# can-lehmann/exprgrad

Hardware: AMD Instinct MI355X
Metric: GFLOP/s matmul 4096^3 f32 (1 GPU) (higher is better)
Workload: dtype f32

## Files before the change

exprgrad_amd/csrc/kernels/gemm_split_bf16.hip:

```cpp
#include <algorithm>
#include <cfloat>

#include "gemm_fused.hpp"
#include "../eg_internal.hpp"
#include "../switches.hpp"

namespace {

typedef __bf16 bf16x8 __attribute__((ext_vector_type(8)));
typedef float f32x4 __attribute__((ext_vector_type(4)));


struct SplitOperand {
  const float* src;
  long ld;
  long R;
  int kc;
  __bf16* dst;
};

__device__ __forceinline__ void unit_coords(const SplitOperand& o, long K, long u, long& r, long& chunk) {
  const long cpr = K / 8, t = u >> 6;
  const int l = (int)(u & 63);
  if (o.kc) {
    const long per = cpr / 4;
    r = (t / per) * 16 + (l >> 2);
    chunk = (t % per) * 4 + (l & 3);
  } else {
    const long per = cpr / 2;
    r = (t / per) * 32 + (l >> 1);
    chunk = (t % per) * 2 + (l & 1);
  }
}

__device__ __forceinline__ void load_unit(const SplitOperand& o, long r, long chunk, float (&x)[8]) {
  if (o.kc) {
    const f32x4* p = reinterpret_cast<const f32x4*>(o.src + r * o.ld + chunk * 8);
    const f32x4 v0 = __builtin_nontemporal_load(p), v1 = __builtin_nontemporal_load(p + 1);
#pragma unroll
    for (int j = 0; j < 4; ++j) {
      x[j] = v0[j];
      x[4 + j] = v1[j];
    }
  } else {
    const float* p = o.src + chunk * 8 * o.ld + r;
#pragma unroll
    for (int j = 0; j < 8; ++j) x[j] = __builtin_nontemporal_load(p + j * o.ld);
  }
}

__device__ __forceinline__ void split_unit(const SplitOperand& o, long K, long r, long chunk, const float (&x)[8], bool& bad) {
  bf16x8 h0, h1, h2;
#pragma unroll
  for (int j = 0; j < 8; ++j) {
    const float v = x[j];
    const __bf16 b0 = (__bf16)v;
    const float r1 = v - (float)b0;
    const __bf16 b1 = (__bf16)r1;
    const float f1 = (float)b1;
    const float r2 = r1 - f1;
    const __bf16 b2 = (__bf16)r2;
    const float f2 = (float)b2;
    bad |= !(r2 == f2);
    bad |= v != 0.f && __builtin_fabsf(v) < FLT_MIN;
    bad |= (f1 != 0.f && __builtin_fabsf(f1) < FLT_MIN) || (f2 != 0.f && __builtin_fabsf(f2) < FLT_MIN);
    h0[j] = b0;
    h1[j] = b1;
    h2[j] = b2;
  }
  const long plane = o.R * K;
  bf16x8* d = reinterpret_cast<bf16x8*>(o.dst + ((chunk >> 1) * o.R + r) * 16 + (chunk & 1) * 8);
  const long ps = plane / 8;
  d[0] = h0;
  d[ps] = h1;
  d[2 * ps] = h2;
}

constexpr int SPLIT_NT = 256;
constexpr int SPLIT_U = 2;

__global__ __launch_bounds__(SPLIT_NT) void split_planes_kernel(SplitOperand a, SplitOperand b, long K, long units_a, long units,
                                                              unsigned* flag, unsigned epoch) {
  constexpr long STEP = (long)SPLIT_NT * SPLIT_U;
  const long per = ((units + gridDim.x - 1) / gridDim.x + STEP - 1) / STEP * STEP;
  const long lo = (long)blockIdx.x * per, hi = lo + per < units ? lo + per : units;
  bool bad = false;
  for (long base = lo; base < hi; base += STEP) {
    float x[SPLIT_U][8];
    long r[SPLIT_U], c[SPLIT_U];
#pragma unroll
    for (int i = 0; i < SPLIT_U; ++i) {
      const long u = base + i * SPLIT_NT + threadIdx.x;
      if (u >= hi) continue;
      const bool in_a = u < units_a;
      unit_coords(in_a ? a : b, K, in_a ? u : u - units_a, r[i], c[i]);
      load_unit(in_a ? a : b, r[i], c[i], x[i]);
    }
#pragma unroll
    for (int i = 0; i < SPLIT_U; ++i) {
      const long u = base + i * SPLIT_NT + threadIdx.x;
      if (u >= hi) continue;
      split_unit(u < units_a ? a : b, K, r[i], c[i], x[i], bad);
    }
  }
  if (__builtin_expect(bad, 0)) *(volatile unsigned*)flag = epoch;
}


constexpr int BM = 256, BN = 256, WM = 128, WN = 64, NT = 512;
constexpr int STAGES = 3;
constexpr int PLANE_BYTES = BM * 16 * 2;
constexpr int STAGE_BYTES = 6 * PLANE_BYTES;
constexpr int LOADS = STAGE_BYTES / (NT * 16);

struct SplitGemmArgs {
  const __bf16* pa;
  const __bf16* pb;
  float* C;
  const float* bias;
  long M, N, K, ldc;
  int tiles_m, tiles_n;
  int accumulate;
  int skew;
  const unsigned* flag;
  unsigned epoch;
};

__device__ __forceinline__ int xcd_remap(int bid, int nwg) {
  constexpr int NXCD = 8;
  const int q = nwg / NXCD, r = nwg % NXCD;
  const int xcd = bid % NXCD, local = bid / NXCD;
  return (xcd < r ? xcd * (q + 1) : r * (q + 1) + (xcd - r) * q) + local;
}
__device__ __forceinline__ void tile_origin(int wgid, int tiles_m, int tiles_n, long& m_blk, long& n_blk) {
  constexpr int GROUP = 8;
  const int per_group = GROUP * tiles_n;
  const int first_m = (wgid / per_group) * GROUP;
  const int gsize = min(tiles_m - first_m, GROUP);
  const int in_group = wgid % per_group;
  m_blk = (long)(first_m + in_group % gsize) * BM;
  n_blk = (long)(in_group / gsize) * BN;
}

__device__ __forceinline__ const void* uniform_ptr(const void* p) {
  const unsigned long v = reinterpret_cast<unsigned long>(p);
  const unsigned lo = __builtin_amdgcn_readfirstlane((unsigned)v), hi = __builtin_amdgcn_readfirstlane((unsigned)(v >> 32));
  return reinterpret_cast<const void*>(((unsigned long)hi << 32) | lo);
}

constexpr int ROLE_LOAD_OWN = 1, ROLE_LOAD_PARTNER = 2, ROLE_READ_TOP = 4, ROLE_READ_AHEAD = 8;
constexpr int PARTNER = 4;

#ifdef EG_SPLIT_GEMM_STAMPS
constexpr int STAMP_BLOCKS = 1024;
__device__ unsigned long long g_split_stamps[STAMP_BLOCKS][8][4];
#define EG_STAMP(t)                                                                  \
  do {                                                                               \
    __builtin_amdgcn_sched_barrier(0);                                               \
    asm volatile("s_memtime %0\n\ts_waitcnt lgkmcnt(0)" : "=s"(t)::"memory"); \
    __builtin_amdgcn_sched_barrier(0);                                               \
  } while (0)
#else
#define EG_STAMP(t) \
  do {              \
  } while (0)
#endif

__global__ __launch_bounds__(NT) void split_gemm_kernel(SplitGemmArgs a) {
  if (*(volatile const unsigned*)a.flag == a.epoch) return;
  __shared__ __attribute__((aligned(16))) unsigned char lds[STAGES * STAGE_BYTES];

  const int tid = threadIdx.x, lane = tid & 63, wave = __builtin_amdgcn_readfirstlane(tid >> 6);
  const int wr = wave >> 2, wc = wave & 3;
  long m_blk, n_blk;
  tile_origin(xcd_remap(blockIdx.x, gridDim.x), a.tiles_m, a.tiles_n, m_blk, n_blk);

  const __amdgpu_buffer_rsrc_t ra = __builtin_amdgcn_make_buffer_rsrc(
      const_cast<void*>(uniform_ptr(a.pa + m_blk * 16)), (short)0, -1, 0x00020000);
  const __amdgpu_buffer_rsrc_t rb = __builtin_amdgcn_make_buffer_rsrc(
      const_cast<void*>(uniform_ptr(a.pb + n_blk * 16)), (short)0, -1, 0x00020000);
  const unsigned a_plane = (unsigned)(a.M * a.K * 2), b_plane = (unsigned)(a.N * a.K * 2);
  const unsigned a_ktile = (unsigned)(a.M * 32), b_ktile = (unsigned)(a.N * 32);
  const unsigned voff = (unsigned)lane * 16;

  auto pieces = [&](int kt, int s, int w) {
    unsigned char* st = lds + s * STAGE_BYTES + w * 1024;
    const unsigned at = (unsigned)kt * a_ktile + (unsigned)w * 1024, bt = (unsigned)kt * b_ktile + (unsigned)w * 1024;
#pragma unroll
    for (int i = 0; i < LOADS; ++i) {
      __attribute__((address_space(3))) void* dst = (__attribute__((address_space(3))) void*)(st + i * PLANE_BYTES);
      if (i < 3)
        __builtin_amdgcn_raw_ptr_buffer_load_lds(ra, dst, 16, voff, (unsigned)i * a_plane + at, 0, 0);
      else
        __builtin_amdgcn_raw_ptr_buffer_load_lds(rb, dst, 16, voff, (unsigned)(i - 3) * b_plane + bt, 0, 0);
    }
  };
  auto issue = [&](int kt, int s, int r) {
    if (r & ROLE_LOAD_OWN) pieces(kt, s, wave);
    if (r & ROLE_LOAD_PARTNER) pieces(kt, s, wave ^ PARTNER);
  };

  f32x4 acc[8][4];
#pragma unroll
  for (int i = 0; i < 8; ++i)
#pragma unroll
    for (int j = 0; j < 4; ++j)
#pragma unroll
      for (int r = 0; r < 4; ++r) acc[i][j][r] = 0.f;

  const int sel = lane >> 5;
  const int a_row = (wr * WM + (lane & 15)) * 32 + ((lane >> 4) & 1) * 16;
  const int b_row = 3 * PLANE_BYTES + (wc * WN + (lane & 15)) * 32 + ((lane >> 4) & 1) * 16;
  const int a01_off = a_row + sel * PLANE_BYTES, a02_off = a_row + 2 * sel * PLANE_BYTES;
  const int b21_off = b_row + (2 - sel) * PLANE_BYTES, b10_off = b_row + (1 - sel) * PLANE_BYTES, b00_off = b_row;

  bf16x8 fb21[4], fb10[4], fb00[4], fa01, fa02;
  auto read_head = [&](const unsigned char* st) {
#pragma unroll
    for (int j = 0; j < 4; ++j) {
      fb21[j] = *reinterpret_cast<const bf16x8*>(st + b21_off + j * 512);
      fb10[j] = *reinterpret_cast<const bf16x8*>(st + b10_off + j * 512);
      fb00[j] = *reinterpret_cast<const bf16x8*>(st + b00_off + j * 512);
    }
    fa01 = *reinterpret_cast<const bf16x8*>(st + a01_off);
    fa02 = *reinterpret_cast<const bf16x8*>(st + a02_off);
  };
#pragma unroll
  for (int j = 0; j < 4; ++j) fb21[j] = fb10[j] = fb00[j] = bf16x8{};
  fa01 = fa02 = bf16x8{};

  const int skew = a.skew;
  const int role = !skew ? ROLE_LOAD_OWN | ROLE_READ_TOP
                         : (wave & PARTNER) ? ROLE_LOAD_OWN | ROLE_LOAD_PARTNER | ROLE_READ_TOP : ROLE_READ_AHEAD;
  const int KT = (int)(a.K / 16);
  issue(0, 0, role);
  if (KT > 1) issue(1, 1, role);
  if (skew) {
    if (KT > 1) asm volatile("s_waitcnt vmcnt(12)" ::: "memory");
    else asm volatile("s_waitcnt vmcnt(0)" ::: "memory");
    __builtin_amdgcn_s_barrier();
    asm volatile("" ::: "memory");
    if (role & ROLE_READ_AHEAD) read_head(lds);
  }
#ifdef EG_SPLIT_GEMM_STAMPS
  unsigned long long t0 = 0, t1 = 0, t2 = 0, front = 0, body = 0, back = 0;
#endif
  int s = 0;
  for (int kt = 0; kt < KT; ++kt) {
    if (!skew && kt + 1 < KT) asm volatile("s_waitcnt vmcnt(6)" ::: "memory");
    else asm volatile("s_waitcnt vmcnt(0)" ::: "memory");
    __builtin_amdgcn_s_barrier();
    asm volatile("" ::: "memory");
#ifdef EG_SPLIT_GEMM_STAMPS
    EG_STAMP(t0);
    if (kt) back += t0 - t2;
#endif
    int r = role;
    asm volatile("" : "+s"(r));
    if (kt + 2 < KT) issue(kt + 2, s == 0 ? 2 : s - 1, r);
    const unsigned char* st = lds + s * STAGE_BYTES;
    if (r & ROLE_READ_TOP) read_head(st);
    EG_STAMP(t1);
    bf16x8 c01 = fa01, c02 = fa02;
#pragma unroll
    for (int i = 0; i < 8; ++i) {
      bf16x8 n01 = c01, n02 = c02;
      __builtin_amdgcn_sched_barrier(0);
      if (i + 1 < 8) {
        n01 = *reinterpret_cast<const bf16x8*>(st + a01_off + (i + 1) * 512);
        n02 = *reinterpret_cast<const bf16x8*>(st + a02_off + (i + 1) * 512);
      }
      __builtin_amdgcn_sched_barrier(0);
#pragma unroll
      for (int j = 0; j < 4; ++j) acc[i][j] = __builtin_amdgcn_mfma_f32_16x16x32_bf16(c01, fb21[j], acc[i][j], 0, 0, 0);
#pragma unroll
      for (int j = 0; j < 4; ++j) acc[i][j] = __builtin_amdgcn_mfma_f32_16x16x32_bf16(c01, fb10[j], acc[i][j], 0, 0, 0);
#pragma unroll
      for (int j = 0; j < 4; ++j) acc[i][j] = __builtin_amdgcn_mfma_f32_16x16x32_bf16(c02, fb00[j], acc[i][j], 0, 0, 0);
      c01 = n01;
      c02 = n02;
    }
    EG_STAMP(t2);
#ifdef EG_SPLIT_GEMM_STAMPS
    front += t1 - t0;
    body += t2 - t1;
#endif
    s = s == STAGES - 1 ? 0 : s + 1;
    if ((r & ROLE_READ_AHEAD) && kt + 1 < KT) read_head(lds + s * STAGE_BYTES);
  }
#ifdef EG_SPLIT_GEMM_STAMPS
  if (lane == 0 && blockIdx.x < STAMP_BLOCKS) {
    unsigned long long* o = g_split_stamps[blockIdx.x][wave];
    o[0] = front;
    o[1] = body;
    o[2] = back;
    o[3] = (unsigned long long)KT;
  }
#endif

  __syncthreads();
  float* park = reinterpret_cast<float*>(lds) + wave * 64 * WN;
  const int prow = lane >> 4, pc4 = (lane & 15) * 4;
  const long col = n_blk + wc * WN + pc4;
  f32x4 b4 = {0.f, 0.f, 0.f, 0.f};
  if (a.bias) b4 = *reinterpret_cast<const f32x4*>(a.bias + col);
#pragma unroll
  for (int h = 0; h < 2; ++h) {
#pragma unroll
    for (int i = 0; i < 4; ++i)
#pragma unroll
      for (int j = 0; j < 4; ++j)
#pragma unroll
        for (int r = 0; r < 4; ++r) park[(i * 16 + 4 * prow + r) * WN + j * 16 + (lane & 15)] = acc[4 * h + i][j][r];
    asm volatile("s_waitcnt lgkmcnt(0)" ::: "memory");
#pragma unroll
    for (int q = 0; q < 16; ++q) {
      const int row = 4 * q + prow;
      f32x4 v = *reinterpret_cast<const f32x4*>(park + row * WN + pc4);
      f32x4* c = reinterpret_cast<f32x4*>(a.C + (m_blk + wr * WM + h * 64 + row) * a.ldc + col);
      if (a.accumulate) v = *c + v;
      if (a.bias) v = v + b4;
      *c = v;
    }
    asm volatile("s_waitcnt lgkmcnt(0)" ::: "memory");
  }
}

inline bool aligned16(const void* p) { return (reinterpret_cast<uintptr_t>(p) & 15) == 0; }

constexpr size_t kPlaneCap = 1ull << 30;

}

namespace eg {
namespace gemm {

int sgemm_split(eg_ctx* ctx, int trans_a, int trans_b, long M, long N, long K, const float* A, long lda, const float* B, long ldb,
                float* C, long ldc, int accumulate, const float* bias) {
  if (!ctx || !A || !B || !C || M <= 0 || N <= 0 || K <= 0) return EG_ERR_UNSUPPORTED;
  if (lda < (trans_a ? M : K) || ldb < (trans_b ? K : N) || ldc < N) return EG_ERR_UNSUPPORTED;
  if (eg::sw::on("EG_NO_SPLIT_GEMM")) return EG_ERR_UNSUPPORTED;
  if (M % BM != 0 || N % BN != 0 || K % 32 != 0 || K < 2048) return EG_ERR_UNSUPPORTED;
  if ((M / BM) * (N / BN) < ctx->compute_units) return EG_ERR_UNSUPPORTED;
  const size_t plane_bytes = 6 * (size_t)(M + N) * (size_t)K;
  if (plane_bytes > kPlaneCap || 6 * (size_t)std::max(M, N) * (size_t)K >= (1ull << 31)) return EG_ERR_UNSUPPORTED;
  if (!aligned16(A) || !aligned16(B) || (!trans_a && lda % 4 != 0) || (trans_b && ldb % 4 != 0)) return EG_ERR_UNSUPPORTED;
  if (!aligned16(C) || ldc % 4 != 0 || (bias && !aligned16(bias))) return EG_ERR_UNSUPPORTED;
  if (!exact_single_launch(ctx, trans_a, trans_b, M, N, K, A, lda, B, ldb, C, ldc, bias)) return EG_ERR_UNSUPPORTED;

  int rc = eg::set_device(ctx);
  if (rc) return rc;
  if (!ctx->split_flag) {
    EG_HIP_CHECK(hipMalloc((void**)&ctx->split_flag, sizeof(unsigned)));
    EG_HIP_CHECK(hipMemset(ctx->split_flag, 0, sizeof(unsigned)));
  }
  rc = eg::ensure_workspace(ctx, plane_bytes);
  if (rc) return rc;
  if (++ctx->split_epoch == 0) ctx->split_epoch = 1;
  const unsigned epoch = ctx->split_epoch;

  __bf16* pa = static_cast<__bf16*>(ctx->workspace);
  __bf16* pb = pa + 3 * (size_t)M * K;
  const SplitOperand oa = {A, lda, M, trans_a ? 0 : 1, pa};
  const SplitOperand ob = {B, ldb, N, trans_b ? 1 : 0, pb};
  const long units_a = M * K / 8, units = (M + N) * K / 8;
  long blocks = (units + SPLIT_NT * SPLIT_U - 1) / (SPLIT_NT * SPLIT_U);
  if (blocks > 8L * ctx->compute_units) blocks = 8L * ctx->compute_units;
  hipLaunchKernelGGL(split_planes_kernel, dim3((unsigned)blocks), dim3(SPLIT_NT), 0, ctx->stream, oa, ob, K, units_a, units,
                     ctx->split_flag, epoch);
  EG_HIP_CHECK(hipGetLastError());

  SplitGemmArgs g = {};
  g.pa = pa;
  g.pb = pb;
  g.C = C;
  g.bias = bias;
  g.M = M;
  g.N = N;
  g.K = K;
  g.ldc = ldc;
  g.tiles_m = (int)(M / BM);
  g.tiles_n = (int)(N / BN);
  g.accumulate = accumulate;
  g.skew = eg::sw::present("EG_GEMM_NO_SKEW") ? 0 : 1;
  g.flag = ctx->split_flag;
  g.epoch = epoch;
  hipLaunchKernelGGL(split_gemm_kernel, dim3((unsigned)(g.tiles_m * g.tiles_n)), dim3(NT), 0, ctx->stream, g);
  EG_HIP_CHECK(hipGetLastError());

  return sgemm_exact(ctx, trans_a, trans_b, M, N, K, A, lda, B, ldb, C, ldc, accumulate, bias, ctx->split_flag, epoch);
}

}
}

#ifdef EG_SPLIT_GEMM_STAMPS
extern "C" int eg_debug_split_stamps(unsigned long long* dst, size_t count) {
  if (count > sizeof(g_split_stamps) / sizeof(unsigned long long)) return EG_ERR_UNSUPPORTED;
  EG_HIP_CHECK(hipDeviceSynchronize());
  EG_HIP_CHECK(hipMemcpyFromSymbol(dst, HIP_SYMBOL(g_split_stamps), count * sizeof(unsigned long long)));
  return 0;
}
#endif
```

Measured before the change: 255,000.

## Interleave A and B split work per block and vectorize bf16 splitting

Rewrites the split pass so each block gets a balanced, interleaved share of A and B work items instead of a contiguous unit range. Hot loads and conversions become cheaper: unit coordinates use 32-bit division, bf16 conversions run two lanes at a time, and the subnormal checks use the hardware class instruction. The aim is to balance memory traffic between the two operands (which have different access patterns) and trim ALU work in a bandwidth-bound preprocessing kernel. It also adds optional timestamp instrumentation behind a compile flag, plus shape checks that reject shapes the partition cannot handle.

```diff
diff --git a/exprgrad_amd/csrc/kernels/gemm_split_bf16.hip b/exprgrad_amd/csrc/kernels/gemm_split_bf16.hip
--- a/exprgrad_amd/csrc/kernels/gemm_split_bf16.hip
+++ b/exprgrad_amd/csrc/kernels/gemm_split_bf16.hip
@@ -2,6 +2,7 @@
 #include <cfloat>
 
 #include "gemm_fused.hpp"
+#include "split_partition.hpp"
 #include "../eg_internal.hpp"
 #include "../switches.hpp"
 
@@ -19,20 +20,6 @@
   __bf16* dst;
 };
 
-__device__ __forceinline__ void unit_coords(const SplitOperand& o, long K, long u, long& r, long& chunk) {
-  const long cpr = K / 8, t = u >> 6;
-  const int l = (int)(u & 63);
-  if (o.kc) {
-    const long per = cpr / 4;
-    r = (t / per) * 16 + (l >> 2);
-    chunk = (t % per) * 4 + (l & 3);
-  } else {
-    const long per = cpr / 2;
-    r = (t / per) * 32 + (l >> 1);
-    chunk = (t % per) * 2 + (l & 1);
-  }
-}
-
 __device__ __forceinline__ void load_unit(const SplitOperand& o, long r, long chunk, float (&x)[8]) {
   if (o.kc) {
     const f32x4* p = reinterpret_cast<const f32x4*>(o.src + r * o.ld + chunk * 8);
@@ -49,24 +36,31 @@
   }
 }
 
+typedef __bf16 bf16x2 __attribute__((ext_vector_type(2)));
+typedef float f32x2 __attribute__((ext_vector_type(2)));
+constexpr unsigned kSubnormal = (1u << 4) | (1u << 7);
+
 __device__ __forceinline__ void split_unit(const SplitOperand& o, long K, long r, long chunk, const float (&x)[8], bool& bad) {
   bf16x8 h0, h1, h2;
 #pragma unroll
-  for (int j = 0; j < 8; ++j) {
-    const float v = x[j];
-    const __bf16 b0 = (__bf16)v;
-    const float r1 = v - (float)b0;
-    const __bf16 b1 = (__bf16)r1;
-    const float f1 = (float)b1;
-    const float r2 = r1 - f1;
-    const __bf16 b2 = (__bf16)r2;
-    const float f2 = (float)b2;
-    bad |= !(r2 == f2);
-    bad |= v != 0.f && __builtin_fabsf(v) < FLT_MIN;
-    bad |= (f1 != 0.f && __builtin_fabsf(f1) < FLT_MIN) || (f2 != 0.f && __builtin_fabsf(f2) < FLT_MIN);
-    h0[j] = b0;
-    h1[j] = b1;
-    h2[j] = b2;
+  for (int j = 0; j < 8; j += 2) {
+    const f32x2 v = {x[j], x[j + 1]};
+    const bf16x2 b0 = __builtin_convertvector(v, bf16x2);
+    const f32x2 r1 = v - __builtin_convertvector(b0, f32x2);
+    const bf16x2 b1 = __builtin_convertvector(r1, bf16x2);
+    const f32x2 f1 = __builtin_convertvector(b1, f32x2);
+    const f32x2 r2 = r1 - f1;
+    const bf16x2 b2 = __builtin_convertvector(r2, bf16x2);
+    const f32x2 f2 = __builtin_convertvector(b2, f32x2);
+#pragma unroll
+    for (int e = 0; e < 2; ++e) {
+      bad |= !(r2[e] == f2[e]);
+      bad |= __builtin_amdgcn_classf(v[e], kSubnormal);
+      bad |= __builtin_amdgcn_classf(f1[e], kSubnormal) || __builtin_amdgcn_classf(f2[e], kSubnormal);
+      h0[j + e] = b0[e];
+      h1[j + e] = b1[e];
+      h2[j + e] = b2[e];
+    }
   }
   const long plane = o.R * K;
   bf16x8* d = reinterpret_cast<bf16x8*>(o.dst + ((chunk >> 1) * o.R + r) * 16 + (chunk & 1) * 8);
@@ -76,34 +70,54 @@
   d[2 * ps] = h2;
 }
 
-constexpr int SPLIT_NT = 256;
+constexpr int SPLIT_NT = eg::gemm::kSplitItemUnits;
 constexpr int SPLIT_U = 2;
 
-__global__ __launch_bounds__(SPLIT_NT) void split_planes_kernel(SplitOperand a, SplitOperand b, long K, long units_a, long units,
+#ifdef EG_SPLIT_PASS_STAMPS
+constexpr int PASS_STAMP_BLOCKS = 4096;
+__device__ unsigned long long g_pass_stamps[PASS_STAMP_BLOCKS][2];
+#endif
+
+__global__ __launch_bounds__(SPLIT_NT) void split_planes_kernel(SplitOperand a, SplitOperand b, long K, eg::gemm::SplitShares shares,
                                                               unsigned* flag, unsigned epoch) {
-  constexpr long STEP = (long)SPLIT_NT * SPLIT_U;
-  const long per = ((units + gridDim.x - 1) / gridDim.x + STEP - 1) / STEP * STEP;
-  const long lo = (long)blockIdx.x * per, hi = lo + per < units ? lo + per : units;
+#ifdef EG_SPLIT_PASS_STAMPS
+  const unsigned long long born = __builtin_amdgcn_s_memrealtime();
+#endif
+  eg::gemm::SplitWalk w = eg::gemm::split_walk(shares, gridDim.x, blockIdx.x);
   bool bad = false;
-  for (long base = lo; base < hi; base += STEP) {
+  while (w.left >= SPLIT_U) {
     float x[SPLIT_U][8];
     long r[SPLIT_U], c[SPLIT_U];
+    int in_b[SPLIT_U];
 #pragma unroll
     for (int i = 0; i < SPLIT_U; ++i) {
-      const long u = base + i * SPLIT_NT + threadIdx.x;
-      if (u >= hi) continue;
-      const bool in_a = u < units_a;
-      unit_coords(in_a ? a : b, K, in_a ? u : u - units_a, r[i], c[i]);
-      load_unit(in_a ? a : b, r[i], c[i], x[i]);
-    }
-#pragma unroll
-    for (int i = 0; i < SPLIT_U; ++i) {
-      const long u = base + i * SPLIT_NT + threadIdx.x;
-      if (u >= hi) continue;
-      split_unit(u < units_a ? a : b, K, r[i], c[i], x[i], bad);
-    }
+      const eg::gemm::SplitItem it = eg::gemm::split_next(w);
+      in_b[i] = it.in_b;
+      eg::gemm::split_unit_coords(it.in_b ? b.kc : a.kc, K, it.item * SPLIT_NT + threadIdx.x, r[i], c[i]);
+    }
+#pragma unroll
+    for (int i = 0; i < SPLIT_U; ++i) load_unit(in_b[i] ? b : a, r[i], c[i], x[i]);
+#pragma unroll
+    for (int i = 0; i < SPLIT_U; ++i) split_unit(in_b[i] ? b : a, K, r[i], c[i], x[i], bad);
+  }
+  while (w.left > 0) {
+    float x[8];
+    long r, c;
+    const eg::gemm::SplitItem it = eg::gemm::split_next(w);
+    const SplitOperand& o = it.in_b ? b : a;
+    eg::gemm::split_unit_coords(o.kc, K, it.item * SPLIT_NT + threadIdx.x, r, c);
+    load_unit(o, r, c, x);
+    split_unit(o, K, r, c, x, bad);
   }
   if (__builtin_expect(bad, 0)) *(volatile unsigned*)flag = epoch;
+#ifdef EG_SPLIT_PASS_STAMPS
+  asm volatile("s_waitcnt vmcnt(0)" ::: "memory");
+  __syncthreads();
+  if (threadIdx.x == 0 && blockIdx.x < PASS_STAMP_BLOCKS) {
+    g_pass_stamps[blockIdx.x][0] = born;
+    g_pass_stamps[blockIdx.x][1] = __builtin_amdgcn_s_memrealtime();
+  }
+#endif
 }
 
 
@@ -363,11 +377,11 @@
   __bf16* pb = pa + 3 * (size_t)M * K;
   const SplitOperand oa = {A, lda, M, trans_a ? 0 : 1, pa};
   const SplitOperand ob = {B, ldb, N, trans_b ? 1 : 0, pb};
-  const long units_a = M * K / 8, units = (M + N) * K / 8;
-  long blocks = (units + SPLIT_NT * SPLIT_U - 1) / (SPLIT_NT * SPLIT_U);
-  if (blocks > 8L * ctx->compute_units) blocks = 8L * ctx->compute_units;
-  hipLaunchKernelGGL(split_planes_kernel, dim3((unsigned)blocks), dim3(SPLIT_NT), 0, ctx->stream, oa, ob, K, units_a, units,
-                     ctx->split_flag, epoch);
+  const long items_a = split_items(M, K), items_b = split_items(N, K);
+  if (items_a < 0 || items_b < 0) return EG_ERR_UNSUPPORTED;
+  const long blocks = split_blocks(items_a, items_b, SPLIT_U, 8L * ctx->compute_units);
+  hipLaunchKernelGGL(split_planes_kernel, dim3((unsigned)blocks), dim3(SPLIT_NT), 0, ctx->stream, oa, ob, K,
+                     split_shares(items_a, items_b, blocks), ctx->split_flag, epoch);
   EG_HIP_CHECK(hipGetLastError());
 
   SplitGemmArgs g = {};
@@ -394,6 +408,15 @@
 }
 }
 
+#ifdef EG_SPLIT_PASS_STAMPS
+extern "C" int eg_debug_split_pass_stamps(unsigned long long* dst, size_t count) {
+  if (count > sizeof(g_pass_stamps) / sizeof(unsigned long long)) return EG_ERR_UNSUPPORTED;
+  EG_HIP_CHECK(hipDeviceSynchronize());
+  EG_HIP_CHECK(hipMemcpyFromSymbol(dst, HIP_SYMBOL(g_pass_stamps), count * sizeof(unsigned long long)));
+  return 0;
+}
+#endif
+
 #ifdef EG_SPLIT_GEMM_STAMPS
 extern "C" int eg_debug_split_stamps(unsigned long long* dst, size_t count) {
   if (count > sizeof(g_split_stamps) / sizeof(unsigned long long)) return EG_ERR_UNSUPPORTED;
diff --git a/exprgrad_amd/csrc/kernels/split_partition.hpp b/exprgrad_amd/csrc/kernels/split_partition.hpp
--- /dev/null
+++ b/exprgrad_amd/csrc/kernels/split_partition.hpp
@@ -0,0 +1,92 @@
+#pragma once
+
+#if defined(__HIP__) || defined(__CUDACC__)
+#define EG_SPLIT_HD __host__ __device__
+#else
+#define EG_SPLIT_HD
+#endif
+
+namespace eg {
+namespace gemm {
+
+constexpr int kSplitItemUnits = 256;
+
+EG_SPLIT_HD inline long split_items(long R, long K) {
+  if (R <= 0 || K <= 0 || R % 32 != 0 || K % 32 != 0) return -1;
+  const long units = R * (K / 8);
+  return units % kSplitItemUnits == 0 ? units / kSplitItemUnits : -1;
+}
+
+EG_SPLIT_HD inline long split_blocks(long items_a, long items_b, long in_flight, long cap) {
+  const long want = (items_a + items_b + in_flight - 1) / in_flight;
+  return want < 1 ? 1 : want < cap ? want : cap;
+}
+
+struct SplitShares {
+  long a_q, a_rem, b_q, b_rem;
+};
+
+EG_SPLIT_HD inline SplitShares split_shares(long items_a, long items_b, long blocks) {
+  SplitShares s;
+  s.a_q = items_a / blocks;
+  s.a_rem = items_a % blocks;
+  s.b_q = items_b / blocks;
+  s.b_rem = items_b % blocks;
+  return s;
+}
+
+struct SplitWalk {
+  long a_next, b_next;
+  long a_n;
+  long n;
+  long left;
+  long acc;
+};
+
+struct SplitItem {
+  int in_b;
+  long item;
+};
+
+EG_SPLIT_HD inline SplitWalk split_walk(const SplitShares& s, long blocks, long block) {
+  SplitWalk w;
+  const long late = block - (blocks - s.b_rem);
+  w.a_next = block * s.a_q + (block < s.a_rem ? block : s.a_rem);
+  w.b_next = block * s.b_q + (late > 0 ? late : 0);
+  w.a_n = s.a_q + (block < s.a_rem ? 1 : 0);
+  w.n = w.a_n + s.b_q + (late >= 0 ? 1 : 0);
+  w.left = w.n;
+  w.acc = 0;
+  return w;
+}
+
+EG_SPLIT_HD inline SplitItem split_next(SplitWalk& w) {
+  SplitItem it;
+  w.acc += w.a_n;
+  if (w.acc >= w.n) {
+    w.acc -= w.n;
+    it.in_b = 0;
+    it.item = w.a_next++;
+  } else {
+    it.in_b = 1;
+    it.item = w.b_next++;
+  }
+  --w.left;
+  return it;
+}
+
+EG_SPLIT_HD inline void split_unit_coords(int kc, long K, long u, long& r, long& chunk) {
+  const unsigned t = (unsigned)(u >> 6), l = (unsigned)(u & 63);
+  const unsigned per = (unsigned)(K >> (kc ? 5 : 4));
+  const unsigned grp = t / per, pos = t - grp * per;
+  if (kc) {
+    r = (long)grp * 16 + (l >> 2);
+    chunk = (long)pos * 4 + (l & 3);
+  } else {
+    r = (long)grp * 32 + (l >> 1);
+    chunk = (long)pos * 2 + (l & 1);
+  }
+}
+
+}
+}
```

Result: no change. 256,700, median of 6 (+0.7%).
